# epfl-lts2/pygsp

Hardware: AMD Instinct MI355X
Metric: filtered-vertices/sec (N·Nsig·K/s) + achieved HBM GB/s vs roofline, 1M-vertex K=30 (higher is better)
Workload: dtype f64

## Files before the change

pygsp_amd/csrc/gspx.hip:

```cpp
#include "gspx_kernels.hip.h"
#include "gspx_tile_kernels.hip.h"

#include <hip/hip_runtime.h>

#include <algorithm>
#include <atomic>
#include <chrono>
#include <cmath>
#include <cstdarg>
#include <cstdio>
#include <cstring>
#include <map>
#include <memory>
#include <numeric>
#include <mutex>
#include <string>
#include <thread>
#include <vector>
#include <sys/mman.h>

#include "../../include/gspx.h"
#include "../../include/gspx_ext.h"

using namespace gspx;
// ... 219 lines not shown
  void destroy() {
    if (st) (void)hipStreamDestroy(st);
    st = nullptr;
    for (auto& e : ev) {
      if (e) (void)hipEventDestroy(e);
      e = nullptr;
    }
    for (auto& pm : pin) pm.release();
    ready = false;
  }
};

struct HostPipe {
  static constexpr int NIN = 3;
  hipStream_t stream_in = nullptr, stream_out = nullptr;
  hipEvent_t h2d_ev[NIN] = {nullptr, nullptr, nullptr};
  hipEvent_t t_in[NIN][2] = {{nullptr, nullptr}, {nullptr, nullptr}, {nullptr, nullptr}};
  hipEvent_t t_out[2] = {nullptr, nullptr};
  PinMem pin_in[NIN], pin_out[2];
  DevMem dx[NIN], dy[2];
  double timing[9] = {0, 0, 0, 0, 0, 0, 0, 0, 0};
  std::vector<double> timeline;
  bool ready = false;
  int init() {
    if (ready) return GSPX_OK;
    HIPCHK(hipStreamCreateWithFlags(&stream_in, hipStreamNonBlocking));
    HIPCHK(hipStreamCreateWithFlags(&stream_out, hipStreamNonBlocking));
    for (auto& e : h2d_ev) HIPCHK(hipEventCreateWithFlags(&e, hipEventDisableTiming));
    for (auto& sl : t_in)
      for (auto& e : sl) HIPCHK(hipEventCreate(&e));
    for (auto& e : t_out) HIPCHK(hipEventCreate(&e));
    ready = true;
    return GSPX_OK;
  }
  void destroy() {
    if (stream_in) (void)hipStreamDestroy(stream_in);
    if (stream_out) (void)hipStreamDestroy(stream_out);
    for (auto& e : h2d_ev)
      if (e) (void)hipEventDestroy(e);
    for (auto& sl : t_in)
      for (auto& e : sl) {
        if (e) (void)hipEventDestroy(e);
        e = nullptr;
      }
    for (auto& e : t_out) {
      if (e) (void)hipEventDestroy(e);
      e = nullptr;
    }
    stream_in = stream_out = nullptr;
    for (auto& e : h2d_ev) e = nullptr;
    for (int i = 0; i < NIN; ++i) {
      pin_in[i].release();
      dx[i].release();
    }
    for (int i = 0; i < 2; ++i) {
      pin_out[i].release();
      dy[i].release();
    }
    ready = false;
  }
};

struct Options {
  int64_t kernel = 0;
  int64_t vec = 0;
  int64_t rows_per_wave = 0;
  int64_t narrow_g_log2 = -1;
  int64_t waves_per_block = 4;
  int64_t calib_mix = 0;
  int64_t graph_launch = 2;
  int64_t tile_gather = 1;
  int64_t tile_workgroups = 0;
  int64_t knn_f32 = 1;
  int64_t tile_pad = 1;
  int64_t tile_min_row = 16;
  int64_t staged_copy = 1;
  int64_t staged_copy_min_mb = 32;
  int64_t copy_threads = 0;
  int64_t tile_regroup = 1;
  int64_t tile_lg = 0;
  int64_t edge_vertex_walk = 1;
  int64_t fuse_input = 1;
  int64_t tile_nt = -1;
  int64_t synthesis = 0;
  int64_t alternate_sweep = 1;
  int64_t xcd_remap = 1;
  int64_t combine = 0;
  int64_t ws_limit_mb = 65536;
  int64_t max_batch = 0;
  int64_t gather_rccl = 1;
  int64_t lds_pad_kb = 0;
  int64_t host_pipeline = 1;
  int64_t host_batch = 0;
  int64_t host_edge = 0;
  int64_t host_threads = 0;
  int64_t streamed_alloc = 1;
};

struct gspx_ctx {
  int device = 0;
  int cu_count = 256;
  hipStream_t stream = nullptr;
  Options opt;
  DevMem ws_t;
  DevMem ws_r;
  DevMem ws_w;
  DevMem io_x, io_y;
  DevMem ws_spec;
  HostPipe* pipe = nullptr;
  CopyStage* copy = nullptr;
  bool counted = false;
  std::mutex comms_mu;
  std::vector<struct gspx_comm*> comms;
  hipEvent_t ev[4] = {nullptr, nullptr, nullptr, nullptr};
  std::vector<hipEvent_t> ev_pool;
  double timing[8] = {0, 0, 0, 0, 0, 0, 0, 0};
  bool capturing = false;
  std::vector<unsigned char> seen_key;
  std::vector<unsigned char> graph_key;
  hipGraphExec_t graph_exec = nullptr;
  const struct BatchProgram* batch_program = nullptr;
};
struct BatchProgram {
  int S;
  const double *sc, *be, *ga;
  bool old_is_x;
};

static std::atomic<int> g_live_ctx[64];

static void replay_reset(gspx_ctx* ctx) {
  if (!ctx) return;
  ctx->seen_key.clear();
  ctx->graph_key.clear();
  if (ctx->graph_exec) {
    (void)hipGraphExecDestroy(ctx->graph_exec);
    ctx->graph_exec = nullptr;
  }
}

struct gspx_buf {
  gspx_ctx* ctx = nullptr;
  DevMem mem;
  int64_t bytes = 0;
};

static std::atomic<uint64_t> g_generation{1};


struct gspx_graph {
  gspx_ctx* ctx = nullptr;
  const uint64_t generation = g_generation.fetch_add(1);
  int64_t N = 0;
  int dtype = GSPX_F64;
  bool from_w = false;
  int64_t nnz_l = 0;
  DevMem lptr, lcol, lval, dw;
  int64_t nnz_int = 0;
  DevMem rptr, rcol, rval, fval, coff;
  unsigned coff_ldb = 0;
  DevMem perm, iperm;
  bool has_perm = false;
  double fval_lmax = -1.0;
  double build_ms = 0.0;
  bool has_bounds = false;
  double bounds[4] = {0, 0, 0, 0};
// ... 63 lines not shown
      ctx->cu_count < 1)
    ctx->cu_count = 256;
  hipError_t e = hipStreamCreateWithFlags(&ctx->stream, hipStreamNonBlocking);
  if (e != hipSuccess) {
    delete ctx;
    return set_err(GSPX_ERR_HIP, "hipStreamCreate failed: %s", hipGetErrorString(e));
  }
  for (int i = 0; i < 4; ++i) {
    e = hipEventCreate(&ctx->ev[i]);
    if (e != hipSuccess) {
      delete ctx;
      return set_err(GSPX_ERR_HIP, "hipEventCreate failed: %s", hipGetErrorString(e));
    }
  }
  *out = ctx;
  return GSPX_OK;
}

static void comm_invalidate_all(gspx_ctx* ctx);

extern "C" int gspx_ctx_destroy(gspx_ctx* ctx) {
  replay_reset(ctx);
  if (!ctx) return GSPX_OK;
  if (ctx->counted) g_live_ctx[ctx->device & 63].fetch_sub(1);
  comm_invalidate_all(ctx);
  if (ctx->graph_exec) {
    (void)hipGraphExecDestroy(ctx->graph_exec);
    ctx->graph_exec = nullptr;
  }
  (void)hipSetDevice(ctx->device);
  if (ctx->stream) (void)hipStreamSynchronize(ctx->stream);
  for (int i = 0; i < 4; ++i)
    if (ctx->ev[i]) (void)hipEventDestroy(ctx->ev[i]);
  for (hipEvent_t e : ctx->ev_pool) (void)hipEventDestroy(e);
  ctx->ws_t.release();
  ctx->ws_r.release();
  ctx->ws_w.release();
  ctx->io_x.release();
  ctx->io_y.release();
  ctx->ws_spec.release();
  if (ctx->pipe) {
    ctx->pipe->destroy();
    delete ctx->pipe;
    ctx->pipe = nullptr;
  }
  if (ctx->copy) {
    ctx->copy->destroy();
    delete ctx->copy;
    ctx->copy = nullptr;
  }
  if (ctx->stream) (void)hipStreamDestroy(ctx->stream);
  delete ctx;
  return GSPX_OK;
}

extern "C" int gspx_ctx_sync(gspx_ctx* ctx) {
  if (!ctx) return set_err(GSPX_ERR_INVALID, "null ctx");
  HIPCHK(hipSetDevice(ctx->device));
  HIPCHK(hipStreamSynchronize(ctx->stream));
  return GSPX_OK;
}

static int64_t* option_slot(Options& o, const char* key) {
  if (!key) return nullptr;
  if (!strcmp(key, "kernel")) return &o.kernel;
  if (!strcmp(key, "vec")) return &o.vec;
  if (!strcmp(key, "rows_per_wave")) return &o.rows_per_wave;
  if (!strcmp(key, "narrow_g_log2")) return &o.narrow_g_log2;
  if (!strcmp(key, "waves_per_block")) return &o.waves_per_block;
  if (!strcmp(key, "alternate_sweep")) return &o.alternate_sweep;
  if (!strcmp(key, "synthesis")) return &o.synthesis;
  if (!strcmp(key, "tile_gather")) return &o.tile_gather;
  if (!strcmp(key, "graph_launch")) return &o.graph_launch;
  if (!strcmp(key, "tile_workgroups")) return &o.tile_workgroups;
  if (!strcmp(key, "tile_lg")) return &o.tile_lg;
  if (!strcmp(key, "tile_regroup")) return &o.tile_regroup;
  if (!strcmp(key, "staged_copy")) return &o.staged_copy;
  if (!strcmp(key, "staged_copy_min_mb")) return &o.staged_copy_min_mb;
  if (!strcmp(key, "copy_threads")) return &o.copy_threads;
  if (!strcmp(key, "tile_min_row")) return &o.tile_min_row;
  if (!strcmp(key, "tile_pad")) return &o.tile_pad;
  if (!strcmp(key, "knn_f32")) return &o.knn_f32;
  if (!strcmp(key, "tile_nt")) return &o.tile_nt;
  if (!strcmp(key, "fuse_input")) return &o.fuse_input;
  if (!strcmp(key, "edge_vertex_walk")) return &o.edge_vertex_walk;
  if (!strcmp(key, "xcd_remap")) return &o.xcd_remap;
  if (!strcmp(key, "combine")) return &o.combine;
  if (!strcmp(key, "ws_limit_mb")) return &o.ws_limit_mb;
  if (!strcmp(key, "max_batch")) return &o.max_batch;
  if (!strcmp(key, "gather_rccl")) return &o.gather_rccl;
  if (!strcmp(key, "lds_pad_kb")) return &o.lds_pad_kb;
  if (!strcmp(key, "host_pipeline")) return &o.host_pipeline;
  if (!strcmp(key, "host_batch")) return &o.host_batch;
  if (!strcmp(key, "host_edge")) return &o.host_edge;
  if (!strcmp(key, "host_threads")) return &o.host_threads;
  if (!strcmp(key, "streamed_alloc")) return &o.streamed_alloc;
  return nullptr;
}

extern "C" int gspx_ctx_set_option(gspx_ctx* ctx, const char* key, int64_t value) {
  replay_reset(ctx);
  if (!ctx) return set_err(GSPX_ERR_INVALID, "null ctx");
  int64_t* s = option_slot(ctx->opt, key);
  if (!s) return set_err(GSPX_ERR_INVALID, "unknown option '%s'", key ? key : "(null)");
  if (!strcmp(key, "rows_per_wave") && (value < 0 || value > 1024))
    return set_err(GSPX_ERR_INVALID, "rows_per_wave must be in [0, 1024] (0 = auto)");
  if (!strcmp(key, "narrow_g_log2") && (value < -1 || value > 6))
    return set_err(GSPX_ERR_INVALID, "narrow_g_log2 must be in [-1, 6] (-1 = auto)");
  if (!strcmp(key, "waves_per_block") && !(value == 4 || value == 8 || value == 16))
    return set_err(GSPX_ERR_INVALID, "waves_per_block must be 4, 8 or 16");
  if (!strcmp(key, "kernel") && !(value == 0 || value == 1 || value == 2 || value == 5))
    return set_err(GSPX_ERR_INVALID, "kernel must be 0 (auto), 1 (panel), 2 (narrow) or 5 (LDS-staged)");
  if (!strcmp(key, "vec") && !(value == 0 || value == 1 || value == 2 || value == 4))
    return set_err(GSPX_ERR_INVALID, "vec must be 0, 1, 2 or 4");
  *s = value;
  if (!strcmp(key, "streamed_alloc")) {
    const bool on = value != 0;
    (void)hipSetDevice(ctx->device);
    for (DevMem* m : {&ctx->ws_t, &ctx->ws_r}) {
      if (!on && m->va_size) {
        (void)hipStreamSynchronize(ctx->stream);
        m->release();
      }
      m->streamed = on;
    }
  }
  return GSPX_OK;
}

extern "C" int gspx_ctx_get_option(gspx_ctx* ctx, const char* key, int64_t* value) {
  if (!ctx || !value) return set_err(GSPX_ERR_INVALID, "null argument");
  if (key && !strcmp(key, "retired_va_mb")) {
    *value = (int64_t)(g_retired_va_bytes.load() >> 20);
    return GSPX_OK;
  }
  int64_t* s = option_slot(ctx->opt, key);
  if (!s) return set_err(GSPX_ERR_INVALID, "unknown option '%s'", key ? key : "(null)");
  *value = *s;
  return GSPX_OK;
}

extern "C" int gspx_buf_alloc(gspx_ctx* ctx, int64_t bytes, gspx_buf** out) {
  if (!ctx || !out || bytes < 0) return set_err(GSPX_ERR_INVALID, "gspx_buf_alloc: bad argument");
  *out = nullptr;
  HIPCHK(hipSetDevice(ctx->device));
  gspx_buf* b = new gspx_buf();
  b->ctx = ctx;
  b->bytes = bytes;
  int rc = b->mem.alloc((size_t)bytes);
  if (rc != GSPX_OK) {
    delete b;
    return rc;
  }
  *out = b;
  return GSPX_OK;
}

extern "C" int gspx_buf_free(gspx_buf* b) {
  if (!b) return GSPX_OK;
  (void)hipSetDevice(b->ctx->device);
  (void)hipStreamSynchronize(b->ctx->stream);
  delete b;
  return GSPX_OK;
}

static int staged_copy(gspx_ctx* ctx, unsigned char* dev, unsigned char* host, size_t bytes, bool to_device) {
// ... 898 lines not shown
  const size_t total = (size_t)N * (ld / VEC);
  const unsigned nb = (unsigned)std::min<size_t>((total + 255) / 256, 16384);
  if (nb == 0) return;
  constexpr int NFB = 8;
  for (int f0 = 0; f0 < nf; f0 += NFB) {
    const int here = std::min(NFB, nf - f0);
    hipLaunchKernelGGL((k_combine<T, VEC, NFB>), dim3(nb), dim3(256), 0, st, slots, nslots,
                       slot_stride, cf, M, f0, here, N, ld, y, ldy, plane_y, perm, 0, pitch);
  }
}

template <typename T>
static void launch_combine(const T* slots, int nslots, size_t slot_stride, const T* cf, int M,
                           int nf, int N, unsigned ld, T* y, unsigned ldy, size_t plane_y,
                           const int* perm, int vec, hipStream_t st, unsigned pitch = 0) {
  if (!pitch) pitch = ld;
  if constexpr (sizeof(T) == 4) {
    if (vec == 4)
      return launch_combine_v<T, 4>(slots, nslots, slot_stride, cf, M, nf, N, ld, y, ldy, plane_y,
                                    perm, st, pitch);
  }
  if (vec == 2)
    return launch_combine_v<T, 2>(slots, nslots, slot_stride, cf, M, nf, N, ld, y, ldy, plane_y,
                                  perm, st, pitch);
  return launch_combine_v<T, 1>(slots, nslots, slot_stride, cf, M, nf, N, ld, y, ldy, plane_y,
                                perm, st, pitch);
}

template <typename T> static int ensure_factor(gspx_graph* g, double lmax) {
  if (g->fval_lmax == lmax) return GSPX_OK;
  gspx_ctx* ctx = g->ctx;
  const int N = (int)g->N;
  const T a1 = (T)(lmax / 2.0), a2 = (T)(lmax / 2.0);
  const T two_over_a1 = T(2) / a1;
  const int nb = std::max(1, (N + 255) / 256);
  if (N > 0)
    hipLaunchKernelGGL((k_factor<T>), dim3(nb), dim3(256), 0, ctx->stream, g->rptr.as<int>(),
                       g->rcol.as<int>(), g->rval.as<T>(), N, two_over_a1, a2, g->fval.as<T>());
  HIPCHK(hipGetLastError());
  g->fval_lmax = lmax;
  return GSPX_OK;
}

static hipEvent_t pool_event(gspx_ctx* ctx, size_t& i_ref) {
  size_t i = i_ref - 1;
  if (i >= 1024) {
    i = 1020 + (i & 3);
    i_ref = i + 1;
  }
  while (ctx->ev_pool.size() <= i) {
    hipEvent_t e = nullptr;
    if (hipEventCreate(&e) != hipSuccess) return nullptr;
    ctx->ev_pool.push_back(e);
  }
  return ctx->ev_pool[i];
}

__global__ void k_s1nat(const int* __restrict__ s1, const int* __restrict__ perm, int n, int* __restrict__ nat) {
  const int i = blockIdx.x * 256 + threadIdx.x;
  if (i < n) nat[i] = perm[s1[i]];
}
static int ensure_s1nat(gspx_graph* g, hipStream_t st) {
  if (g->gt_s1nat.p || !g->has_perm) return GSPX_OK;
  CHK(g->gt_s1nat.alloc((size_t)std::max(g->gt_ns1, 1) * 4 + 64));
  if (g->gt_ns1 > 0)
    hipLaunchKernelGGL(k_s1nat, dim3((g->gt_ns1 + 255) / 256), dim3(256), 0, st, g->gt_s1rows.as<int>(),
                       g->perm.as<int>(), g->gt_ns1, g->gt_s1nat.as<int>());
  return GSPX_OK;
}

template <typename T> static bool tile_geometry(const gspx_graph* g, const Options& opt, unsigned ld) {
  constexpr int TVEC = 16 / (int)sizeof(T);
  const size_t U = (size_t)g->N * ld;
  return opt.tile_gather && g->gt_rows == GSPX_TILE_BR && (size_t)ld * sizeof(T) >= (size_t)opt.tile_min_row &&
         (ld % TVEC) == 0 && U * sizeof(T) < ((size_t)1 << 31) && (size_t)g->nnz_int * sizeof(T) < ((size_t)1 << 31);
}
template <typename T>
static bool tile_usable(const gspx_graph* g, const Options& opt, unsigned ld, const T* y, unsigned ldy) {
  constexpr int TVEC = 16 / (int)sizeof(T);
  return tile_geometry<T>(g, opt, ld) && (ldy % TVEC) == 0 && (((uintptr_t)y / sizeof(T)) % TVEC) == 0;
}
template <typename T>
static int launch_step_tile(gspx_graph* g, const Options& opt, TileArgs<T> t, unsigned ld, hipStream_t st,
                            const T* vals = nullptr) {
  const size_t rowb = (size_t)ld * sizeof(T);
  int lg = rowb <= 16 ? 1 : rowb <= 32 ? 2 : rowb <= 64 ? 4 : rowb <= 128 ? 8 : 16;
  if (opt.tile_lg == 8 || opt.tile_lg == 4 || opt.tile_lg == 2) lg = rowb <= 128 ? std::max(lg, (int)opt.tile_lg) : 16;
  const bool narrow = lg < 16;
  const int ncol = narrow ? 1 : (int)((rowb + 255) / 256);
  const int flavour = t.old_rows ? 1 : t.nin > 0 ? 2 : 0;
  typedef void (*kern_t)(const TileArgs<T>);
  static const kern_t wide[3][3] = {
      {k_step_tile<T, 0>, k_step_tile<T, 1>, k_step_tile<T, 2>},
      {k_step_tile<T, 0, 16, true>, k_step_tile<T, 1, 16, true>, k_step_tile<T, 2, 16, true>},
      {k_step_tile<T, 0, 16, false, true>, k_step_tile<T, 1, 16, false, true>, k_step_tile<T, 2, 16, false, true>}};
  static const kern_t slim[3][4] = {
      {k_step_tile<T, 1, 1, false, false, 64>, k_step_tile<T, 1, 2, false, false, 128>,
       k_step_tile<T, 1, 4, false, false, 256>, k_step_tile<T, 1, 8>},
      {k_step_tile<T, 1, 1, true, false, 64>, k_step_tile<T, 1, 2, true, false, 128>,
       k_step_tile<T, 1, 4, true, false, 256>, k_step_tile<T, 1, 8, true>},
      {k_step_tile<T, 1, 1, false, true, 64>, k_step_tile<T, 1, 2, false, true, 128>,
       k_step_tile<T, 1, 4, false, true, 256>, k_step_tile<T, 1, 8, false, true>}};
  kern_t kern = narrow ? slim[flavour][lg == 1 ? 0 : lg == 2 ? 1 : lg == 4 ? 2 : 3] : wide[flavour][ncol <= 2 ? ncol : 0];
  unsigned threads = narrow ? 64u * (unsigned)lg : 512u;
  bool mix = false;
  if (opt.calib_mix && !narrow && flavour == 0) {
    static const kern_t mixk[2][3] = {
        {k_step_tile<T, 0, 16, false, false, 512, 16, 1>, k_step_tile<T, 1, 16, false, false, 512, 16, 1>,
         k_step_tile<T, 2, 16, false, false, 512, 16, 1>},
        {k_step_tile<T, 0, 16, false, false, 512, 16, 2>, k_step_tile<T, 1, 16, false, false, 512, 16, 2>,
         k_step_tile<T, 2, 16, false, false, 512, 16, 2>}};
    kern = mixk[opt.calib_mix == 2 ? 1 : 0][ncol <= 2 ? ncol : 0];
    mix = true;
  }
  const int pieces = (int)(rowb / 16);
  if (opt.tile_regroup && ncol == 1 && flavour != 1 && pieces < lg && !mix) {
#define GSPX_CL(LG_, CL_, NT_) \
  (flavour == 2 ? (kern_t)k_step_tile<T, 1, LG_, false, true, NT_, CL_> : (kern_t)k_step_tile<T, 1, LG_, false, false, NT_, CL_>)
    kern_t k2 = nullptr;
    unsigned nt2 = 0;
    if (lg == 4 && pieces == 3) k2 = GSPX_CL(4, 3, 192), nt2 = 192;
    else if (lg == 8 && pieces == 5) k2 = GSPX_CL(8, 5, 320), nt2 = 320;
    else if (lg == 16 && pieces == 10) k2 = GSPX_CL(16, 10, 320), nt2 = 320;
#undef GSPX_CL
    if (k2) kern = k2, threads = nt2;
  }
  size_t lds = g->gt_lds;
  if (lg < 8)
    lds = std::min(lds, (size_t)GSPX_TILE_MAXN1 * 16 * lg + (((size_t)g->gt_entmax * sizeof(T) + 15) & ~(size_t)15) +
                            (((size_t)g->gt_entmax + 15) & ~(size_t)15) + 64);
  if (lg < 8) lds = (lds + 2047) & ~(size_t)2047;
  int per_cu = 2;
  {
    struct Known { size_t attr = 0; std::map<size_t, int> fit; };
    static std::map<std::pair<const void*, int>, Known> known;
    static std::mutex lds_mu;
    std::lock_guard<std::mutex> lock(lds_mu);
    Known& k = known[std::make_pair((const void*)kern, g->ctx->device)];
    if (k.attr < lds) {
      HIPCHK(hipFuncSetAttribute((const void*)kern, hipFuncAttributeMaxDynamicSharedMemorySize, (int)lds));
      k.attr = lds;
    }
    if (lg < 8) {
      auto it = k.fit.find(lds);
      if (it == k.fit.end()) {
        int fit = 2;
        HIPCHK(hipOccupancyMaxActiveBlocksPerMultiprocessor(&fit, (const void*)kern, (int)threads, lds));
        it = k.fit.emplace(lds, std::max(2, std::min(fit, 16))).first;
      }
      per_cu = it->second;
    }
  }
  t.rowptr = g->rptr.as<int>();
  t.col = g->rcol.as<int>();
  t.val = vals ? vals : g->fval.as<T>();
  t.hdr = g->gt_hdr.as<int>();
  if (!t.s1rows) t.s1rows = g->gt_s1rows.as<int>();
  t.lidx = g->gt_lidx.as<unsigned char>();
  t.N = (int)g->N;
  t.ld = ld;
  t.panel_bytes = (unsigned)((size_t)g->N * ld * sizeof(T));
  t.val_bytes = (unsigned)((size_t)g->nnz_int * sizeof(T));
  t.lidx_bytes = (unsigned)((size_t)g->nnz_int);
  t.nb = g->gt_nb;
  t.ncol = ncol;
  t.per_xcd = (t.nb + 7) / 8;
  t.lds_bytes = (int)lds;
  unsigned nwg = (unsigned)std::max<int64_t>(8, ((int64_t)per_cu * g->ctx->cu_count) / 8 * 8);
  if (opt.tile_workgroups > 0)
    nwg = (unsigned)std::max<int64_t>(8, std::min<int64_t>(opt.tile_workgroups, 1 << 20) / 8 * 8);
  nwg = std::min(nwg, 8u * (unsigned)std::max(t.per_xcd, 1));
  t.nt = opt.tile_nt >= 0 ? (int)opt.tile_nt : ((size_t)g->N * ld * sizeof(T) >= ((size_t)192 << 20) ? 5 : 0);
  hipLaunchKernelGGL(kern, dim3(nwg), dim3(threads), lds, st, t);
  return GSPX_OK;
}

template <typename T>
static int prepare_coff(gspx_graph* g, const Shape& shape, unsigned ld, hipStream_t st) {
  if (shape.kernel == 5 && g->coff_ldb != ld * (unsigned)sizeof(T)) {
    CHK(g->coff.ensure(((size_t)g->nnz_int + 64) * sizeof(unsigned)));
    const int nb = std::max(1, (int)((g->N + 255) / 256));
    hipLaunchKernelGGL((k_coff<T>), dim3(nb), dim3(256), 0, st, g->rptr.as<int>(), g->rcol.as<int>(), (int)g->N,
                       ld * (unsigned)sizeof(T), g->coff.as<unsigned>());
    g->coff_ldb = ld * (unsigned)sizeof(T);
  }
  return GSPX_OK;
}


template <typename T>
static int run_batch(gspx_graph* g, int nf, int M, const std::vector<double>& cp, const T* x,
                     unsigned ldx, T* y, unsigned ldy, unsigned ld, bool deferred,
                     bool acc_existing, bool final_to_y, size_t& ev_idx) {
  gspx_ctx* ctx = g->ctx;
  const Options& opt = ctx->opt;
  hipStream_t st = ctx->stream;
  const int N = (int)g->N;
  const int K = M - 1;
  constexpr unsigned TVEC = 16 / (unsigned)sizeof(T);
  const unsigned ldp = (ld + TVEC - 1) / TVEC * TVEC;
  const bool tile_direct = (deferred || nf == 1) && tile_usable<T>(g, opt, ld, y, ldy);
  const bool pad_pays = opt.tile_pad == 2 || ld >= 2 ||
                        (size_t)g->nnz_int * (sizeof(T) + 4) >= ((size_t)20 << 20);
  const bool padded = !tile_direct && (deferred || nf == 1) && opt.tile_pad && pad_pays && tile_geometry<T>(g, opt, ldp);
  const unsigned ldw = padded ? ldp : ld;
  const size_t U = (size_t)N * ldw;
  int veccap = 4;
  while (veccap > 1 && ((ldy % veccap) != 0 || (((uintptr_t)y / sizeof(T)) % veccap) != 0))
// ... 400 lines not shown
      a.gamma = has_b2 ? T(-1) : T(0);
      a.scale = (k == 0) ? T(0.5) : T(1);
    }
    a.reverse = (opt.alternate_sweep && (k & 1)) ? 1 : 0;
    launch_step<T>(a, shape, opt, st, g->coff.as<unsigned>());
  }
  HIPCHK(hipEventRecord(e2, st));
  if (padded) {
    const unsigned nbp = (unsigned)std::min<size_t>(((size_t)N * ld + 255) / 256, 65536);
    hipLaunchKernelGGL((k_permute_out_pad<T>), dim3(nbp), dim3(256), 0, st, B[0], ldw, y, ldy, ld, N, perm);
  }
  HIPCHK(hipEventRecord(e3, st));
  HIPCHK(hipGetLastError());
  return GSPX_OK;
}

template <typename T>
static int run_batch_program(gspx_graph* g, int S, const double* sc, const double* be, const double* ga, bool old_is_x,
                             const T* x, unsigned ldx, T* y, unsigned ldy, unsigned ld, size_t& ev_idx) {
  gspx_ctx* ctx = g->ctx;
  Options opt = ctx->opt;
  hipStream_t st = ctx->stream;
  const int N = (int)g->N;
  const size_t U = (size_t)N * ld;
  int veccap = 4;
  while (veccap > 1 && ((ldy % veccap) != 0 || (((uintptr_t)y / sizeof(T)) % veccap) != 0))
    veccap /= 2;
  const Shape shape = choose_shape(opt, sizeof(T), ld, veccap);
  const int* perm = g->has_perm ? g->perm.as<int>() : nullptr;

  const T hw[3] = {T(1), T(0), T(0)};
  CHK(ctx->ws_w.ensure(sizeof(hw) + 64));
  HIPCHK(hipMemcpyAsync(ctx->ws_w.p, hw, sizeof(hw), hipMemcpyHostToDevice, st));
  HIPCHK(hipStreamSynchronize(st));
  CHK(ctx->ws_t.ensure((old_is_x ? 3 : 2) * U * sizeof(T) + 256));
  T* X = ctx->ws_t.as<T>();
  T* H[2] = {X + U, old_is_x ? X + 2 * U : X};

  hipEvent_t e0 = pool_event(ctx, ++ev_idx), e1 = pool_event(ctx, ++ev_idx),
             e2 = pool_event(ctx, ++ev_idx), e3 = pool_event(ctx, ++ev_idx);
  if (!e0 || !e1 || !e2 || !e3) return set_err(GSPX_ERR_HIP, "hipEventCreate failed");
  HIPCHK(hipEventRecord(e0, st));
  int pvec = shape.vec;
  while (pvec > 1 && ((ldx % pvec) != 0 || (((uintptr_t)x / sizeof(T)) % pvec) != 0)) pvec /= 2;
  launch_permute_in<T>(x, ldx, X, ld, N, perm, pvec, st);
  HIPCHK(hipEventRecord(e1, st));

  CHK(prepare_coff<T>(g, shape, ld, st));
  StepArgs<T> a{};
  a.rowptr = g->rptr.as<int>();
  a.col = g->rcol.as<int>();
  a.val = g->fval.as<T>();
  a.N = N;
  a.ld = ld;
  a.curbytes = (u32)(U * sizeof(T));
  a.nf = 1;
  a.racc = H[0];
  a.y = y;
  a.ldy = ldy;
  a.perm = perm;
  a.wts = ctx->ws_w.as<T>();
  const bool tile_ok = tile_usable<T>(g, opt, ld, y, ldy);
  for (int s = 0; s < S; ++s) {
    const bool last = s == S - 1;
    const T* cur = (s == 0) ? X : H[(s - 1) & 1];
    T* out = H[s & 1];
    const T* old = old_is_x ? X : (const T*)out;
    const double gam = (!old_is_x && s == 0) ? 0.0 : ga[s];
    if (tile_ok) {
      TileArgs<T> t{};
      t.cur = cur;
      t.old = gam == 0.0 ? cur : old;
      t.out = out;
      t.racc = H[0];
      t.y = y;
      t.ldy = ldy;
      t.perm = perm;
      t.scale = (T)sc[s];
      t.beta = (T)be[s];
      t.gamma = (T)gam;
      t.flush = 0;
      t.final = last ? 1 : 0;
      t.reverse = (opt.alternate_sweep && (s & 1)) ? 1 : 0;
      CHK(launch_step_tile<T>(g, opt, t, ld, st));
      continue;
    }
    a.cur = cur;
    a.old = gam == 0.0 ? cur : old;
    a.out = out;
    a.scale = (T)sc[s];
    a.beta = (T)be[s];
    a.gamma = (T)gam;
    a.flush = last ? 1 : 0;
    a.final = last ? 1 : 0;
    a.reverse = (opt.alternate_sweep && (s & 1)) ? 1 : 0;
    launch_step<T>(a, shape, opt, st, g->coff.as<unsigned>());
  }
  HIPCHK(hipEventRecord(e2, st));
  HIPCHK(hipEventRecord(e3, st));
  HIPCHK(hipGetLastError());
  return GSPX_OK;
}

template <typename T>
static int program_dev_t(gspx_graph* g, double lmax, int S, const double* sc, const double* be, const double* ga,
                         bool old_is_x, int64_t Nsig, const T* x, T* y) {
  gspx_ctx* ctx = g->ctx;
  const Options& opt = ctx->opt;
  const int64_t N = g->N;
  for (int i = 0; i < 5; ++i) ctx->timing[i] = 0;
  if (N == 0 || Nsig == 0) return GSPX_OK;
  CHK(ensure_factor<T>(g, lmax));
  const size_t rowb = (size_t)N * sizeof(T);
  int64_t max_ld = (int64_t)((((size_t)1 << 31) - 65536) / rowb);
  if (max_ld < 1)
    return set_err(GSPX_ERR_INVALID, "graph too large: one signal column exceeds 2 GiB");
  const size_t budget = (size_t)std::max<int64_t>(opt.ws_limit_mb, 1) << 20;
  max_ld = std::min<int64_t>(max_ld, std::max<int64_t>(1, (int64_t)(budget / (rowb * 3))));
  if (opt.max_batch > 0) max_ld = std::min<int64_t>(max_ld, opt.max_batch);
  if (max_ld < Nsig && max_ld >= 4) max_ld &= ~(int64_t)3;
  size_t ev_idx = 0;
  HIPCHK(hipEventRecord(ctx->ev[0], ctx->stream));
  for (int64_t c0 = 0; c0 < Nsig; c0 += max_ld) {
    const unsigned ld = (unsigned)std::min<int64_t>(max_ld, Nsig - c0);
    CHK(run_batch_program<T>(g, S, sc, be, ga, old_is_x, x + c0, (unsigned)Nsig, y + c0, (unsigned)Nsig, ld, ev_idx));
  }
  HIPCHK(hipEventRecord(ctx->ev[1], ctx->stream));
  HIPCHK(hipStreamSynchronize(ctx->stream));
  float ms = 0;
  HIPCHK(hipEventElapsedTime(&ms, ctx->ev[0], ctx->ev[1]));
  ctx->timing[0] = ms;
  double t_perm = 0, t_steps = 0;
  for (size_t i = 0; i + 3 < ev_idx; i += 4) {
    float p = 0, q = 0;
    HIPCHK(hipEventElapsedTime(&p, ctx->ev_pool[i], ctx->ev_pool[i + 1]));
    HIPCHK(hipEventElapsedTime(&q, ctx->ev_pool[i + 1], ctx->ev_pool[i + 2]));
    t_perm += p;
    t_steps += q;
  }
  ctx->timing[1] = t_steps;
  ctx->timing[2] = (double)(ev_idx / 4) * S;
  ctx->timing[3] = t_perm;
  return GSPX_OK;
}

template <typename T>
static int newton_dev_t(gspx_graph* g, double lmax, int K, const double* nodes, const double* dc,
                        int64_t Nsig, const T* x, T* y) {
  std::vector<double> sc((size_t)K), be((size_t)K), ga((size_t)K);
  for (int s = 0; s < K; ++s) {
    const int j = K - 1 - s;
    if (s == 0) {
      sc[0] = 0.5 * dc[K];
      be[0] = 0.0;
      ga[0] = dc[j] - dc[K] * nodes[j];
    } else {
      sc[(size_t)s] = 0.5;
      be[(size_t)s] = -nodes[j];
      ga[(size_t)s] = dc[j];
    }
  }
  return program_dev_t<T>(g, lmax, K, sc.data(), be.data(), ga.data(), true, Nsig, x, y);
}

extern "C" int gspx_poly_program_dev(gspx_graph* g, double lmax, int S, const double* scale, const double* beta,
                                     const double* gamma, int old_is_x, int64_t Nsig, const void* x_dev, void* y_dev,
                                     double* kernel_ms) {
// ... 629 lines not shown
```

pygsp_amd/csrc/gspx_tile_kernels.hip.h:

```cpp
#pragma once

#include "gspx_kernels.hip.h"

namespace gspx {

template <typename T> struct TileArgs {
  const int* rowptr;
  const int* col;
  const T* val;
  const int* hdr;
  const int* s1rows;
  const u8* lidx;
  const T* cur;
  const T* old;
  const int* old_rows;
  T* out;
  T* racc;
  T* y;
  const int* perm;
  int N;
  u32 ld, ldy;
  u32 panel_bytes, val_bytes, lidx_bytes;
  int nb, ncol, per_xcd;
  int lds_bytes;
  T scale, gamma;
  T beta;
  T wn, wc, wo;
  const T* inp;
  const T* wts;
  int nin;
  int flush;
  int final;
  int reverse;
  int nt;
};

constexpr int GSPX_TILE_BR = 64;
constexpr int GSPX_TILE_MAXN1 = 160;

template <typename T, int NCOL, int LG, bool OLDNAT> struct TileSchedule {
  static constexpr bool PF = !OLDNAT;
  static constexpr bool TILE_LAST = PF && LG == 16;
  static constexpr bool PF_ENTRIES = PF;
  static constexpr bool META_AFTER = !OLDNAT && LG == 16 && NCOL == 0;
};

template <typename T, int NCOL, int LG = 16, bool OLDNAT = false, bool INS = false, int NT = 512, int CL = LG,
          int MIX = 0>
__global__ __launch_bounds__(NT, 4) void k_step_tile(const TileArgs<T> a) {
  static_assert(NT == 512 || (NT == 64 * LG && NCOL == 1) || (CL < LG && NCOL == 1 && NT % 64 == 0 && NT % CL == 0),
                "narrow builds: one row per group, one chunk per row");
  constexpr int BR = GSPX_TILE_BR;
  static_assert(CL <= LG && (BR % (NT / CL)) == 0, "compute groups must tile the block's rows");
  constexpr int MAXN1 = GSPX_TILE_MAXN1;
  constexpr bool PF = TileSchedule<T, NCOL, LG, OLDNAT>::PF;
  constexpr bool META_AFTER = TileSchedule<T, NCOL, LG, OLDNAT>::META_AFTER;
  constexpr bool TILE_LAST = TileSchedule<T, NCOL, LG, OLDNAT>::TILE_LAST;
  constexpr bool PF_ENTRIES = TileSchedule<T, NCOL, LG, OLDNAT>::PF_ENTRIES;
  constexpr int VEC = 16 / (int)sizeof(T);
  typedef typename VT<T, VEC>::t V;
  typedef __attribute__((address_space(3))) void* lds_ptr;
  extern __shared__ __attribute__((aligned(16))) unsigned char gspx_smem[];

  const int tid = threadIdx.x;
  constexpr int NGD = NT / LG;
  constexpr int NG = NT / CL;
  constexpr int NE = (512 + NT - 1) / NT;
  constexpr int RPG = BR / NG;
  constexpr int ST = (MAXN1 + NGD - 1) / NGD;
  constexpr int RB = LG * 16;
  const int lane_d = tid & (LG - 1);
  const int grp_d = tid / LG;
  const int lane16 = CL == LG ? lane_d : tid % CL;
  const int grp = CL == LG ? grp_d : tid / CL;
  const int wave = tid >> 6;
  const int nwx = (int)(gridDim.x >> 3);
  const int xlo = (int)(blockIdx.x & 7) * a.per_xcd;
  int k1 = xlo + a.per_xcd;
  if (k1 > a.nb) k1 = a.nb;
  const int k0 = xlo + (int)(blockIdx.x >> 3);
  if (k0 >= k1) return;

  constexpr u32 POISON = 0x80000000u;
  const rsrc_t rcur = __builtin_amdgcn_make_buffer_rsrc((void*)a.cur, 0, a.panel_bytes, 0x00020000);
  const rsrc_t rold = __builtin_amdgcn_make_buffer_rsrc((void*)a.old, 0, a.panel_bytes, 0x00020000);
  const rsrc_t rra = __builtin_amdgcn_make_buffer_rsrc((void*)a.racc, 0, a.panel_bytes, 0x00020000);
  const rsrc_t rv = __builtin_amdgcn_make_buffer_rsrc((void*)a.val, 0, a.val_bytes, 0x00020000);
  const rsrc_t ri = __builtin_amdgcn_make_buffer_rsrc((void*)a.lidx, 0, a.lidx_bytes, 0x00020000);
  const u32 ldb = a.ld * (u32)sizeof(T);

  struct Meta { int rows[ST]; int rp[RPG + 1]; int orow[OLDNAT ? RPG : 1]; };
  const int xflip = xlo + k1 - 1;
  const bool rev = a.reverse != 0;
  auto phys = [&](int p) { return rev ? xflip - p : p; };
  auto load_hdr = [&](int p) { return *(const int4*)(a.hdr + (size_t)phys(p) * 4); };
  auto uniform = [](int4 h) {
    int4 u;
    u.x = __builtin_amdgcn_readfirstlane(h.x); u.y = __builtin_amdgcn_readfirstlane(h.y);
    u.z = __builtin_amdgcn_readfirstlane(h.z); u.w = __builtin_amdgcn_readfirstlane(h.w);
    return u;
  };
  auto load_meta = [&](int k, const int4& h) {
    Meta m;
    const int n1 = h.y;
#pragma unroll
    for (int t = 0; t < ST; ++t) {
      const int u = grp_d + NGD * t;
      m.rows[t] = a.s1rows[h.x + (u < n1 ? u : 0)];
    }
    int r = phys(k) * BR + grp * RPG;
#pragma unroll
    for (int t = 0; t < RPG + 1; ++t) m.rp[t] = a.rowptr[(r + t) <= a.N ? (r + t) : a.N];
    if constexpr (OLDNAT) {
#pragma unroll
      for (int t = 0; t < RPG; ++t) m.orow[t] = a.old_rows[(r + t) < a.N ? (r + t) : a.N - 1];
    }
    return m;
  };
  V* const tile = (V*)gspx_smem;
  auto stage = [&](const Meta& m, int n1, u32 cb) {
#pragma unroll
    for (int t = 0; t < ST; ++t) {
      if (grp_d + NGD * t < n1)
        __builtin_amdgcn_raw_ptr_buffer_load_lds(rcur, (lds_ptr)(gspx_smem + (wave * (64 / LG) + NGD * t) * RB), 16,
                                                 (u32)m.rows[t] * ldb + cb, 0, 0, 0);
    }
  };
  auto chunk_off_d = [&](int c) {
    const u32 col0 = (c * LG + lane_d) * VEC;
    return col0 < a.ld ? col0 * (u32)sizeof(T) : POISON;
  };
  auto chunk_off = [&](int c) {
// ... 336 lines not shown
```

Measured before the change: 187.9 billion.

## Add two-panel software-pipelined tile kernel for the first Chebyshev step

Adds a specialised tile SpMM kernel variant that double-buffers headers, metadata, entries and the gathered input tile across blocks, prefetching the next panel while computing the current one. It is used only for the plain wide flavour when gamma is zero and there is no flush, which in the recurrence means the s==0 step. The aim is to hide gather and metadata latency behind compute for that step. The cost is extra register pressure from holding prefetched metadata and tile vectors, plus a separate code path that has to be maintained.

```diff
diff --git a/pygsp_amd/csrc/gspx.hip b/pygsp_amd/csrc/gspx.hip
--- a/pygsp_amd/csrc/gspx.hip
+++ b/pygsp_amd/csrc/gspx.hip
@@ -325,6 +325,7 @@
   int64_t edge_vertex_walk = 1;
   int64_t fuse_input = 1;
   int64_t tile_nt = -1;
+  int64_t tile_two_panel = 1;
   int64_t synthesis = 0;
   int64_t alternate_sweep = 1;
   int64_t xcd_remap = 1;
@@ -554,6 +555,7 @@
   if (!strcmp(key, "tile_pad")) return &o.tile_pad;
   if (!strcmp(key, "knn_f32")) return &o.knn_f32;
   if (!strcmp(key, "tile_nt")) return &o.tile_nt;
+  if (!strcmp(key, "tile_two_panel")) return &o.tile_two_panel;
   if (!strcmp(key, "fuse_input")) return &o.fuse_input;
   if (!strcmp(key, "edge_vertex_walk")) return &o.edge_vertex_walk;
   if (!strcmp(key, "xcd_remap")) return &o.xcd_remap;
@@ -1618,7 +1620,7 @@
 }
 template <typename T>
 static int launch_step_tile(gspx_graph* g, const Options& opt, TileArgs<T> t, unsigned ld, hipStream_t st,
-                            const T* vals = nullptr) {
+                            const T* vals = nullptr, bool two_panel = false) {
   const size_t rowb = (size_t)ld * sizeof(T);
   int lg = rowb <= 16 ? 1 : rowb <= 32 ? 2 : rowb <= 64 ? 4 : rowb <= 128 ? 8 : 16;
   if (opt.tile_lg == 8 || opt.tile_lg == 4 || opt.tile_lg == 2) lg = rowb <= 128 ? std::max(lg, (int)opt.tile_lg) : 16;
@@ -1660,6 +1662,12 @@
     else if (lg == 16 && pieces == 10) k2 = GSPX_CL(16, 10, 320), nt2 = 320;
 #undef GSPX_CL
     if (k2) kern = k2, threads = nt2;
+  }
+  if (two_panel && opt.tile_two_panel && !narrow && flavour == 0 && !mix && threads == 512 && (ncol == 1 || ncol == 2) &&
+      t.gamma == T(0) && t.flush == 0) {
+    static const kern_t two[2] = {k_step_tile<T, 1, 16, false, false, 512, 16, 0, true>,
+                                  k_step_tile<T, 2, 16, false, false, 512, 16, 0, true>};
+    kern = two[ncol - 1];
   }
   size_t lds = g->gt_lds;
   if (lg < 8)
@@ -2226,7 +2234,7 @@
       t.flush = 0;
       t.final = last ? 1 : 0;
       t.reverse = (opt.alternate_sweep && (s & 1)) ? 1 : 0;
-      CHK(launch_step_tile<T>(g, opt, t, ld, st));
+      CHK(launch_step_tile<T>(g, opt, t, ld, st, nullptr, true));
       continue;
     }
     a.cur = cur;
diff --git a/pygsp_amd/csrc/gspx_tile_kernels.hip.h b/pygsp_amd/csrc/gspx_tile_kernels.hip.h
--- a/pygsp_amd/csrc/gspx_tile_kernels.hip.h
+++ b/pygsp_amd/csrc/gspx_tile_kernels.hip.h
@@ -45,9 +45,247 @@
   static constexpr bool META_AFTER = !OLDNAT && LG == 16 && NCOL == 0;
 };
 
+template <typename T, int NCOL>
+__device__ __forceinline__ void step_tile_two(const TileArgs<T>& a) {
+  static_assert(NCOL == 1 || NCOL == 2, "two-panel build: one or two column chunks");
+  constexpr int LG = 16, NT = 512, BR = GSPX_TILE_BR, MAXN1 = GSPX_TILE_MAXN1;
+  constexpr int NG = NT / LG;
+  constexpr int RPG = BR / NG;
+  constexpr int ST = (MAXN1 + NG - 1) / NG;
+  constexpr int VEC = 16 / (int)sizeof(T);
+  constexpr int RB = LG * 16;
+  typedef typename VT<T, VEC>::t V;
+  typedef __attribute__((address_space(3))) void* lds_ptr;
+  extern __shared__ __attribute__((aligned(16))) unsigned char gspx_smem[];
+  constexpr u32 POISON = 0x80000000u;
+
+  const int tid = threadIdx.x;
+  const int lane = tid & (LG - 1), grp = tid / LG, wave = tid >> 6;
+  const int nwx = (int)(gridDim.x >> 3);
+  const int xlo = (int)(blockIdx.x & 7) * a.per_xcd;
+  const int k1 = min(xlo + a.per_xcd, a.nb);
+  const int k0 = xlo + (int)(blockIdx.x >> 3);
+  if (k0 >= k1) return;
+
+  const rsrc_t rcur = __builtin_amdgcn_make_buffer_rsrc((void*)a.cur, 0, a.panel_bytes, 0x00020000);
+  const rsrc_t rv = __builtin_amdgcn_make_buffer_rsrc((void*)a.val, 0, a.val_bytes, 0x00020000);
+  const rsrc_t ri = __builtin_amdgcn_make_buffer_rsrc((void*)a.lidx, 0, a.lidx_bytes, 0x00020000);
+  const rsrc_t rout = __builtin_amdgcn_make_buffer_rsrc((void*)a.out, 0, a.panel_bytes, 0x00020000);
+  const u32 ldb = a.ld * (u32)sizeof(T);
+  const int xflip = xlo + k1 - 1;
+  const bool rev = a.reverse != 0;
+  auto phys = [&](int p) { return rev ? xflip - p : p; };
+  auto load_hdr = [&](int p) { return *(const int4*)(a.hdr + (size_t)phys(p) * 4); };
+  auto uniform = [](int4 h) {
+    int4 u;
+    u.x = __builtin_amdgcn_readfirstlane(h.x); u.y = __builtin_amdgcn_readfirstlane(h.y);
+    u.z = __builtin_amdgcn_readfirstlane(h.z); u.w = __builtin_amdgcn_readfirstlane(h.w);
+    return u;
+  };
+  struct Meta { int rows[ST]; int rp[RPG + 1]; };
+  auto load_meta = [&](int k, const int4& h) {
+    Meta m;
+#pragma unroll
+    for (int t = 0; t < ST; ++t) {
+      const int u = grp + NG * t;
+      m.rows[t] = a.s1rows[h.x + (u < h.y ? u : 0)];
+    }
+    const int r = phys(k) * BR + grp * RPG;
+#pragma unroll
+    for (int t = 0; t < RPG + 1; ++t) m.rp[t] = a.rowptr[(r + t) <= a.N ? (r + t) : a.N];
+    return m;
+  };
+  auto chunk_off = [&](int c) {
+    const u32 col0 = (c * LG + lane) * VEC;
+    return col0 < a.ld ? col0 * (u32)sizeof(T) : POISON;
+  };
+  V* const tile = (V*)gspx_smem;
+  u32x4 ev = 0, ei = 0;
+  auto load_entries = [&](const int4& h) {
+    const int nv16 = (h.w * (int)sizeof(T) + 15) >> 4, ni16 = (h.w + 15) >> 4;
+    const bool on = h.y >= 0;
+    const u32 vo = on && tid < nv16 ? (u32)h.z * (u32)sizeof(T) + tid * 16u : POISON;
+    const u32 io = on && tid < ni16 ? (u32)h.z + tid * 16u : POISON;
+    if (a.nt & 1) {
+      ev = __builtin_amdgcn_raw_buffer_load_b128(rv, vo, 0, 2);
+      ei = __builtin_amdgcn_raw_buffer_load_b128(ri, io, 0, 2);
+    } else {
+      ev = __builtin_amdgcn_raw_buffer_load_b128(rv, vo, 0, 0);
+      ei = __builtin_amdgcn_raw_buffer_load_b128(ri, io, 0, 0);
+    }
+  };
+  auto write_entries = [&](const int4& h) {
+    if (h.y < 0) return;
+    T* const mval = (T*)(tile + h.y * LG);
+    u8* const midx = (u8*)(mval + h.w);
+    const int nv16 = (h.w * (int)sizeof(T) + 15) >> 4, ni16 = (h.w + 15) >> 4;
+    if (tid < nv16) *(u32x4*)((unsigned char*)mval + tid * 16) = ev;
+    if (tid < ni16) *(u32x4*)((unsigned char*)midx + tid * 16) = ei;
+    for (int i = tid + NT; i < nv16; i += NT)
+      *(u32x4*)((unsigned char*)mval + i * 16) =
+          __builtin_amdgcn_raw_buffer_load_b128(rv, (u32)h.z * (u32)sizeof(T) + i * 16u, 0, 0);
+    for (int i = tid + NT; i < ni16; i += NT)
+      *(u32x4*)((unsigned char*)midx + i * 16) = __builtin_amdgcn_raw_buffer_load_b128(ri, (u32)h.z + i * 16u, 0, 0);
+  };
+  V sv[ST];
+  auto load_tile = [&](const int* rows, int n1, u32 cb) {
+#pragma unroll
+    for (int t = 0; t < ST; ++t)
+      sv[t] = VT<T, VEC>::bload(rcur, (grp + NG * t < n1 && cb != POISON) ? (u32)rows[t] * ldb + cb : POISON);
+  };
+  auto write_tile = [&](int n1) {
+#pragma unroll
+    for (int t = 0; t < ST; ++t)
+      if (grp + NG * t < n1) tile[(grp + NG * t) * LG + lane] = sv[t];
+  };
+
+  int k = k0, kn = k0 + nwx, knn = k0 + 2 * nwx, k3 = k0 + 3 * nwx;
+  int4 H = uniform(load_hdr(k0));
+  Meta M = load_meta(k0, H);
+  int4 Hn = uniform(load_hdr(kn < k1 ? kn : k0));
+  Meta Mn;
+  int4 Hnn = Hn, Hv = Hn;
+  if constexpr (NCOL == 1) {
+    Mn = load_meta(kn < k1 ? kn : k0, Hn);
+    Hnn = uniform(load_hdr(knn < k1 ? knn : k0));
+    Hv = load_hdr(k3 < k1 ? k3 : k0);
+  }
+  int rs[RPG + 1];
+  load_entries(H);
+  if (H.y >= 0) {
+    const u32 cb = chunk_off(0);
+#pragma unroll
+    for (int t = 0; t < ST; ++t)
+      if (grp + NG * t < H.y)
+        __builtin_amdgcn_raw_ptr_buffer_load_lds(rcur, (lds_ptr)(gspx_smem + (wave * (64 / LG) + NG * t) * RB), 16,
+                                                 cb == POISON ? POISON : (u32)M.rows[t] * ldb + cb, 0, 0, 0);
+  }
+  write_entries(H);
+  __builtin_amdgcn_s_waitcnt(0x0070);
+
+  auto pass = [&](const int c, const bool last) __attribute__((always_inline)) {
+    const int n1 = H.y, rp0 = H.z;
+    const bool fast = n1 >= 0;
+    const T* const mval = (const T*)(tile + (fast ? n1 : 0) * LG);
+    const u8* const midx = (const u8*)(mval + H.w);
+    const int row0 = phys(k) * BR + grp * RPG;
+    if (c == 0) {
+#pragma unroll
+      for (int t = 0; t < RPG + 1; ++t) rs[t] = M.rp[t] & ~3;
+    }
+    const u32 col0 = (c * LG + lane) * VEC;
+    const bool on = col0 < a.ld;
+    const u32 cb = on ? col0 * (u32)sizeof(T) : POISON;
+    asm volatile("" ::: "memory");
+    __builtin_amdgcn_s_waitcnt(0xC07F);
+    __builtin_amdgcn_s_barrier();
+    asm volatile("" ::: "memory");
+    __builtin_amdgcn_sched_barrier(0);
+    const bool more = !last || kn < k1;
+    const int4 none = make_int4(0, -1, 0, 0);
+    int4 Hq = Hnn;
+    if constexpr (NCOL == 2) {
+      if (!last) {
+        int rows[ST];
+#pragma unroll
+        for (int t = 0; t < ST; ++t) rows[t] = M.rows[t];
+        M = load_meta(kn < k1 ? kn : k, Hn);
+        load_tile(rows, n1, chunk_off(1));
+      } else {
+        Hv = load_hdr(knn < k1 ? knn : k);
+        load_tile(M.rows, more ? Hn.y : -1, chunk_off(0));
+        load_entries(more ? Hn : none);
+      }
+    } else {
+      Hq = uniform(Hv);
+      const Meta Mc = Mn;
+      Mn = load_meta(knn < k1 ? knn : k, Hnn);
+      Hv = load_hdr(k3 + nwx < k1 ? k3 + nwx : k);
+      load_tile(Mc.rows, more ? Hn.y : -1, chunk_off(0));
+      load_entries(more ? Hn : none);
+      M = Mc;
+    }
+    __builtin_amdgcn_sched_barrier(0);
+    const V zero = 0;
+    V nv[RPG];
+#pragma unroll
+    for (int t = 0; t < RPG; ++t) {
+      const int s = rs[t], e = rs[t + 1];
+      V acc = 0, self = 0;
+      if (fast) {
+        acc = lds_row_dot<T, V, LG, u8>(mval + (s - rp0), midx + (s - rp0), row0 + t < a.N ? e - s : 0, tile, lane,
+                                        self);
+      } else if (row0 + t < a.N) {
+        for (int j = s; j < e; ++j) {
+          const int cc = a.col[j];
+          const V xv = VT<T, VEC>::bload(rcur, cc < a.N ? (u32)cc * ldb + cb : POISON);
+          if (j == s) self = xv;
+          acc += a.val[j] * xv;
+        }
+      }
+      nv[t] = a.scale * acc + a.gamma * zero + a.beta * self;
+    }
+    asm volatile("" ::: "memory");
+    __builtin_amdgcn_s_waitcnt(0xC07F);
+    __builtin_amdgcn_s_barrier();
+    asm volatile("" ::: "memory");
+    __builtin_amdgcn_sched_barrier(0);
+    if (!a.final) {
+#pragma unroll
+      for (int t = 0; t < RPG; ++t) {
+        const u32 off = (row0 + t < a.N && on) ? (u32)(row0 + t) * ldb + cb : POISON;
+        __builtin_amdgcn_raw_buffer_store_b128(__builtin_bit_cast(u32x4, nv[t]), rout, off, 0, 0);
+      }
+      __builtin_amdgcn_sched_barrier(0);
+    }
+    if (more) {
+      write_tile(last ? Hn.y : n1);
+      if (last) write_entries(Hn);
+    }
+    if (a.final) {
+      __builtin_amdgcn_sched_barrier(0);
+#pragma unroll
+      for (int t = 0; t < RPG; ++t) {
+        const int row = row0 + t;
+        if (row < a.N && on) {
+          const size_t orow = a.perm ? (size_t)a.perm[row] : (size_t)row;
+          *(V*)(a.y + orow * a.ldy + col0) = nv[t];
+        }
+      }
+    }
+    if (last) {
+      H = Hn;
+      if constexpr (NCOL == 2) {
+        Hn = uniform(Hv);
+      } else {
+        Hn = Hnn;
+        Hnn = Hq;
+      }
+      k = kn;
+      kn = knn;
+      knn = k3;
+      k3 += nwx;
+    }
+    return more;
+  };
+  for (;;) {
+    if constexpr (NCOL == 1) {
+      if (!pass(0, true)) break;
+    } else {
+      pass(0, false);
+      if (!pass(1, true)) break;
+    }
+  }
+}
+
 template <typename T, int NCOL, int LG = 16, bool OLDNAT = false, bool INS = false, int NT = 512, int CL = LG,
-          int MIX = 0>
+          int MIX = 0, bool TWO = false>
 __global__ __launch_bounds__(NT, 4) void k_step_tile(const TileArgs<T> a) {
+  if constexpr (TWO) {
+    static_assert(LG == 16 && NT == 512 && CL == 16 && !OLDNAT && !INS && !MIX, "two-panel build: wide, plain");
+    step_tile_two<T, NCOL>(a);
+    return;
+  }
   static_assert(NT == 512 || (NT == 64 * LG && NCOL == 1) || (CL < LG && NCOL == 1 && NT % 64 == 0 && NT % CL == 0),
                 "narrow builds: one row per group, one chunk per row");
   constexpr int BR = GSPX_TILE_BR;
```

Result: no change. 187.4 billion, median of 6 (-0.2%).
